# morriscb/chomp

Hardware: AMD Instinct MI355X
Metric: halo-model P(k,z) samples/sec (Stage K set-up + Stage E grid) (higher is better)
Workload: dtype f64

## Files before the change

### chomp_amd/csrc/chomp_capi.hip

```cpp
#include <hip/hip_runtime.h>

#include <dlfcn.h>

#include <algorithm>
#include <cmath>
#include <cstdio>
#include <cstddef>
#include <cstdint>
#include <cstdlib>
#include <cstring>
#include <string>
#include <map>
#include <unordered_map>
#include <vector>

#include "../../include/chomp_mi355x.h"
#include "chomp_power_kernels.h"
#include "chomp_proj_kernels.h"
#include "chomp_cov_kernels.h"
#include "chomp_probe_kernel.h"
#include "chomp_de_kernels.h"
#include "chomp_pt_kernels.h"
#include "chomp_tri_kernels.h"
#include "chomp_profile_kernels.h"
// ... 851 lines not shown
    return CHOMP_OK;
  if (n < 4 || n > 240) return fail(ctx, CHOMP_ERR_ARG, "dark energy: cosmo_npoints must be 4..240");
  if (nk > 65535) return fail(ctx, CHOMP_ERR_ARG, "dark energy: more than 65535 distinct (w0, wa)");
  T.valid = false;
  int rc = de_knots(ctx);
  if (rc) return rc;
  const DePar* before = T.d_par;
  rc = ensure(ctx, &T.d_par, &T.cap_par, nk);
  if (rc) return rc;
  if (T.d_par != before) T.sh_par.reset();
  rc = ensure(ctx, &T.d_tab, &T.cap_tab, nk * (size_t)de_stride(n));
  if (rc) return rc;
  rc = upload(ctx, T.d_par, keys.data(), nk * sizeof(DePar), T.sh_par);
  if (rc) return rc;
  hipLaunchKernelGGL(k_de_table, dim3((unsigned)n, (unsigned)nk), dim3(64 * kDeNW), 0, ctx->stream,
                     ctx->cfg, T.d_par, ctx->d_de_knots, T.d_tab);
  hipLaunchKernelGGL(k_de_spline, dim3((unsigned)nk), dim3(64), (size_t)(11 * n) * sizeof(double),
                     ctx->stream, ctx->cfg, T.d_tab);
  HIPCHK(hipGetLastError());
  T.keys = keys;
  T.valid = true;
  return CHOMP_OK;
}

int chomp_set_dark_energy(chomp_ctx* ctx, int on) {
  if (!ctx) return CHOMP_ERR_ARG;
  ctx->dark_energy = on != 0;
  return CHOMP_OK;
}

int chomp_set_general_profile(chomp_ctx* ctx, int on) {
  if (!ctx) return CHOMP_ERR_ARG;
  ctx->general_profile = on != 0;
  return CHOMP_OK;
}

int chomp_get_de_table(chomp_ctx* ctx, int source, size_t index, int what, double* out, size_t n) {
  if (!ctx || !out) return fail(ctx, CHOMP_ERR_ARG, "get_de_table: bad args");
  const int np = ctx->cfg.cosmo_npoints;
  int off;
  size_t want = (size_t)np;
  switch (what) {
    case CHOMP_DE_LN_A: off = de_off_ln_a(np); break;
    case CHOMP_DE_PRESSURE: off = de_off_p(np); break;
    case CHOMP_DE_LEVELS: off = de_off_level(np); break;
    case CHOMP_DE_CONVERGED: off = de_off_conv(np); break;
    case CHOMP_DE_PP: off = de_off_pp(np); want = 4 * (size_t)(np - 1); break;
    default: return fail(ctx, CHOMP_ERR_ARG, "get_de_table: unknown table part");
  }
  if (n != want) return fail(ctx, CHOMP_ERR_ARG, "get_de_table: n must be cosmo_npoints (4 (cosmo_npoints - 1) for the coefficients)");
  HIPCHK(hipSetDevice(ctx->device));
  const double* src;
  if (source == CHOMP_DE_EPOCH) {
    if (!ctx->have_epochs || index >= ctx->n_epoch) return fail(ctx, CHOMP_ERR_STATE, "get_de_table: epoch");
    if (index >= ctx->de_slot.size() || ctx->de_slot[index] < 0)
      return fail(ctx, CHOMP_ERR_STATE, "get_de_table: the epoch's cosmology has no dark energy");
    src = ctx->de_ep.d_tab + (size_t)ctx->de_slot[index] * de_stride(np);
  } else if (source == CHOMP_DE_PROJ) {
    if (!ctx->proj.me_ready || !ctx->proj.de)
      return fail(ctx, CHOMP_ERR_STATE, "get_de_table: no projection set-up with dark energy");
    { const int rcj = proj_join(ctx); if (rcj) return rcj; }
    src = ctx->de_proj.d_tab;
  } else {
    return fail(ctx, CHOMP_ERR_ARG, "get_de_table: unknown source");
  }
  HIPCHK(hipStreamSynchronize(ctx->stream));
  HIPCHK(hipMemcpy(out, src + off, n * sizeof(double), hipMemcpyDeviceToHost));
  return CHOMP_OK;
}

int chomp_epochs_set(chomp_ctx* ctx, size_t n_epoch, const chomp_cosmo* cosmo,
                     const double* z) {
  StageRange range_(ctx, "chomp:epochs_set (Stage K: sigma tables, mass-limit search)");
  if (!ctx || !cosmo || !z || n_epoch == 0) return fail(ctx, CHOMP_ERR_ARG, "epochs_set: bad args");
  for (size_t i = 0; i < n_epoch; ++i) {
    if (!ctx->dark_energy && has_dark_energy(cosmo[i].w0, cosmo[i].wa))
      return fail(ctx, CHOMP_ERR_SCOPE,
                  "w0 != -1 or wa != 0: dynamical dark energy (cosmology.py:96-104) needs "
                  "chomp_set_dark_energy(ctx, 1)");
    if (!(cosmo[i].omega_m0 > 0.0) || !(cosmo[i].h > 0.0) || !(cosmo[i].sigma_8 > 0.0))
      return fail(ctx, CHOMP_ERR_ARG, "epochs_set: omega_m0, h, sigma_8 must be > 0");
  }
  HIPCHK(hipSetDevice(ctx->device));
  int rc = alloc_epochs(ctx, n_epoch);
  if (rc) return rc;
  ctx->n_epoch = n_epoch;
  ctx->status_mirrored = false;
  { const int rch = ensure_hstatus(ctx); if (rch) return rch; }
  ctx->have_mass = ctx->have_halo = false;
  ctx->fam_mask = 0;
  ctx->put_mask.assign(n_epoch, 0u);
  ctx->delta_b_zero = true;
  ctx->have_halofit.assign(n_epoch, 0);
  ctx->tri_built.assign(n_epoch, 0);
  ctx->tri4_built.assign(n_epoch, 0);
  ctx->prof_general.assign(n_epoch, 0);
  rc = upload(ctx, ctx->d_cosmo, cosmo, n_epoch * sizeof(chomp_cosmo), ctx->sh_cosmo);
  if (rc) return rc;
  rc = upload(ctx, ctx->d_z, z, n_epoch * sizeof(double), ctx->sh_z);
  if (rc) return rc;
  std::vector<int> slot(n_epoch), first;
  {
    std::unordered_multimap<uint64_t, int> seen;
    seen.reserve(n_epoch * 2);
    for (size_t i = 0; i < n_epoch; ++i) {
      uint64_t h = 1469598103934665603ull;
      const unsigned char* b = reinterpret_cast<const unsigned char*>(&cosmo[i]);
      for (size_t j = 0; j < sizeof(chomp_cosmo); ++j) { h ^= b[j]; h *= 1099511628211ull; }
      int s_found = -1;
      auto range = seen.equal_range(h);
      for (auto it = range.first; it != range.second; ++it)
        if (std::memcmp(&cosmo[first[it->second]], &cosmo[i], sizeof(chomp_cosmo)) == 0) {
          s_found = it->second;
          break;
        }
      if (s_found < 0) {
        s_found = (int)first.size();
        first.push_back((int)i);
        seen.emplace(h, s_found);
      }
      slot[i] = s_found;
    }
  }
  const size_t n_slots = first.size();
  ctx->n_slots = n_slots;
  ctx->slot = slot;
  first.resize(n_epoch, 0);
  rc = upload(ctx, ctx->d_slot, slot.data(), n_epoch * sizeof(int), ctx->sh_slot);
  if (rc) return rc;
  rc = upload(ctx, ctx->d_first, first.data(), n_epoch * sizeof(int), ctx->sh_first);
  if (rc) return rc;
  std::vector<DePar> de_keys;
  ctx->de_slot.assign(n_epoch, -1);
  if (ctx->dark_energy) {
    std::map<std::pair<double, double>, int> seen;
    for (size_t i = 0; i < n_epoch; ++i) {
      if (!has_dark_energy(cosmo[i].w0, cosmo[i].wa)) continue;
      auto it = seen.emplace(std::make_pair(cosmo[i].w0, cosmo[i].wa), (int)de_keys.size());
      if (it.second) de_keys.push_back(DePar{cosmo[i].w0, cosmo[i].wa});
      ctx->de_slot[i] = it.first->second;
    }
  }
  const bool any_de = !de_keys.empty();
  if (any_de) {
    rc = de_build(ctx, ctx->de_ep, de_keys);
    if (rc) return rc;
    const int* before = ctx->d_de_slot;
    rc = ensure(ctx, &ctx->d_de_slot, &ctx->cap_de_slot, n_epoch);
    if (rc) return rc;
    if (ctx->d_de_slot != before) ctx->sh_de_slot.reset();
    rc = upload(ctx, ctx->d_de_slot, ctx->de_slot.data(), n_epoch * sizeof(int), ctx->sh_de_slot);
    if (rc) return rc;
  }
  const unsigned gy = (unsigned)(n_slots + (n_epoch + 255) / 256);
  rc = with_flag(ctx->with_bao, n_slots >= 16, [&](auto BAO, auto MANY) {
    constexpr int NPT = MANY ? 4 : 1;
    hipLaunchKernelGGL((k_sigma_nodes<BAO, NPT>),
                       dim3(sigma_node_blocks<NPT>() + sigma_lns_blocks<NPT>() + sigma_gtab_blocks<NPT>(), gy),
                       dim3(256), 0, ctx->stream, ctx->cfg, ctx->d_cosmo, ctx->d_z, ctx->d_first,
                       ctx->d_slot, (int)n_slots, (int)n_epoch, ctx->d_epochs, ctx->d_snodes,
                       ctx->d_status);
    if (!MANY) return CHOMP_OK;
    const size_t shl = BAO ? 0 : (size_t)kGTabCount * sizeof(double);
    if constexpr (!BAO) {
      const int rcl = lds_opt_in(ctx, &k_sigma_lns<BAO>, (int)shl);
      if (rcl) return rcl;
    }
    hipLaunchKernelGGL(k_sigma_lns<BAO>, dim3((unsigned)n_slots), dim3(kLnsThreads), shl, ctx->stream,
                       ctx->cfg, ctx->d_cosmo, ctx->d_z, ctx->d_first, ctx->d_snodes);
    return CHOMP_OK;
  });
  if (rc) return rc;
  if (any_de)
    hipLaunchKernelGGL(k_de_epochs, dim3((unsigned)((n_epoch + 63) / 64)), dim3(64), 0, ctx->stream,
                       ctx->cfg, ctx->d_de_slot, (int)n_epoch, ctx->de_ep.d_tab, ctx->d_epochs,
                       ctx->d_status);
  if (n_epoch >= 128)
    with_flag(ctx->with_bao, [&](auto BAO) {
      hipLaunchKernelGGL((k_epoch_probe<BAO, 1, 1>), dim3((unsigned)n_epoch, 2 * kProbes), dim3(64), 0,
                         ctx->stream, ctx->cfg, ctx->d_epochs, ctx->d_search, ctx->d_cand, ctx->d_snodes,
                         ctx->d_probe, ctx->d_count, ctx->d_status);
    });
  chomp::launch_epoch_probe(ctx->with_bao != 0, (unsigned)n_epoch, ctx->stream, ctx->cfg,
                            ctx->d_epochs, ctx->d_search, ctx->d_cand, ctx->d_snodes,
                            ctx->d_probe, ctx->d_count, ctx->d_status);
  if (any_de)
    hipLaunchKernelGGL(k_de_chi, dim3((unsigned)n_epoch), dim3(64), 0, ctx->stream, ctx->cfg,
                       ctx->d_de_slot, ctx->de_ep.d_tab, ctx->d_epochs);
  HIPCHK(hipGetLastError());
  ctx->have_epochs = true;
  return CHOMP_OK;
}

struct HaloPlan {
  unsigned fam = 0, kmask = 0;
  int groups[4] = {-1, -1, -1, -1};
  int ng = 0;
  int want_nbar = 1;
  bool eval = false;
  bool general = false;
  bool has_hod() const {
    return group_hod(groups[0]) || group_hod(groups[1]) || group_hod(groups[2]) ||
           group_hod(groups[3]);
  }
};
static std::vector<chomp_hod_model> zheng_models(const chomp_hod_par* hod, size_t n) {
  std::vector<chomp_hod_model> m(n);
  for (size_t i = 0; i < n; ++i) {
    m[i] = chomp_hod_model{};
    m[i].kind = CHOMP_HOD_ZHENG;
    m[i].zheng = hod[i];
  }
  return m;
}
static_assert(kHodZheng == CHOMP_HOD_ZHENG && kHodMandelbaum == CHOMP_HOD_MANDELBAUM,
              "chomp_math.h's model numbers are the header's");
static_assert(PT_FS2 == CHOMP_PT_FS2 && PT_FS2_LEN == CHOMP_PT_FS2_LEN &&
                  PT_FS2_KDIFF == CHOMP_PT_FS2_KDIFF && PT_FS3 == CHOMP_PT_FS3 &&
                  PT_FS3_PARALLELOGRAM == CHOMP_PT_FS3_PARALLELOGRAM && PT_F3 == CHOMP_PT_F3 &&
                  PT_FS3_BCGS == CHOMP_PT_FS3_BCGS && PT_BISPECTRUM == CHOMP_PT_BISPECTRUM &&
                  PT_BISPECTRUM_LEN == CHOMP_PT_BISPECTRUM_LEN &&
                  PT_TRISPECTRUM == CHOMP_PT_TRISPECTRUM &&
                  PT_TRISPECTRUM_PARALLELOGRAM == CHOMP_PT_TRISPECTRUM_PARALLELOGRAM &&
                  kPtForms == CHOMP_PT_TRISPECTRUM_PARALLELOGRAM + 1,
              "chomp_pt_kernels.h's form numbers are the header's");
static int halo_prepare(chomp_ctx* ctx, const chomp_halo_par* profile, const chomp_hod_model* hod,
                        unsigned tables, HaloPlan* P) {
  const size_t n = ctx->n_epoch;
  for (size_t i = 0; i < n; ++i) {
    if (profile[i].alpha == -1.0) continue;
    if (!ctx->general_profile)
      return fail(ctx, CHOMP_ERR_SCOPE,
                  "halo alpha != -1: the general-profile transform y_general "
                  "(halo.py:491-559) is outside the hot-path scope (NFW only) unless "
                  "chomp_set_general_profile(ctx, 1)");
    if (!(profile[i].alpha > -3.0) || !(profile[i].alpha <= kProfileAlphaMax))
      return fail(ctx, CHOMP_ERR_ARG, "halo_setup: alpha must lie in (-3, 3.5]");
    P->general = true;
  }
  for (size_t i = 0; i < n; ++i)
    if ((hod[i].kind != CHOMP_HOD_ZHENG && hod[i].kind != CHOMP_HOD_MANDELBAUM) ||
        hod[i].reserved != 0)
      return fail(ctx, CHOMP_ERR_ARG, "halo_setup: unknown HOD model");
  std::vector<HodDev> hd(n);
  for (size_t i = 0; i < n; ++i) {
    HodDev& d = hd[i];
    d.model = hod[i].kind;
    d.pad_ = 0;
    d.w = 0.0;
    d.M_min = 0.0;
    if (hod[i].kind == CHOMP_HOD_MANDELBAUM) {
      d.log_M_0 = hod[i].log_M_0;
      mandelbaum_constants(hod[i].log_M_0, &d.log_M_min, &d.M_min);
      d.w = hod[i].w;
      d.sigma = 0.0; d.log_M_1p = 0.0; d.alpha = 1.0;
      d.first_zero = d.second_zero = d.safe_norm = -1.0;
      continue;
    }
    const chomp_hod_par& h = hod[i].zheng;
    d.log_M_min = h.log_M_min; d.sigma = h.sigma; d.log_M_0 = h.log_M_0;
    d.log_M_1p = h.log_M_1p; d.alpha = h.alpha;
    d.first_zero = std::pow(10.0, h.log_M_min +
                                      h.sigma * erfinv_host(2.0 * ctx->cfg.halo_precision - 1.0));
    d.second_zero = std::pow(10.0, h.log_M_0);
    d.safe_norm = std::pow(10.0, h.log_M_min + 1.0 * h.sigma);
    if (h.alpha != 1.0) P->eval = true;
  }
  int rcu = upload(ctx, ctx->d_profile, profile, n * sizeof(chomp_halo_par), ctx->sh_profile);
  if (rcu) return rcu;
  rcu = upload(ctx, ctx->d_hod, hd.data(), n * sizeof(HodDev), ctx->sh_hod);
  if (rcu) return rcu;
  P->fam = tables & ((1u << kFamilies) - 1u);
  P->kmask = P->fam | ((tables & CHOMP_T_EXCLUSION) ? kMaskExclusion : 0u);
  P->ng = 0;
  if (P->fam & ((1u << F_HM) | (1u << F_PPMM))) P->groups[P->ng++] = 0;
  if (P->fam & ((1u << F_HG) | (1u << F_PPGM))) P->groups[P->ng++] = 1;
  if (P->fam & (1u << F_PPGG)) P->groups[P->ng++] = 2;
  if (P->fam & (1u << F_I12)) P->groups[P->ng++] = 3;
  if (P->has_hod() && ctx->cfg.divmax > kNodeLevel)
    P->kmask |= kMaskDeepNodes;
  return CHOMP_OK;
}

static int launch_nu_mass(chomp_ctx* ctx, int mf_kind, const HaloPlan* plan) {
  ctx->status_mirrored = false;
  const size_t n = ctx->n_epoch;
  const TabLayout& L = ctx->L;
  const int ef = (ctx->n_slots < 16 || n > 65535) ? 1 : 0;
  ctx->have_b2 = false;
  if (ctx->second_order) {
    ctx->B2 = make_b2_layout(L.NM);
    const int rcb = ensure(ctx, &ctx->d_b2, &ctx->cap_b2, n * (size_t)ctx->B2.stride);
    if (rcb) return rcb;
  }
  with_flag(ctx->with_bao, (size_t)L.NM * n <= 512, [&](auto BAO, auto FEW) {
    constexpr int NW = FEW ? 4 : 1;
    const dim3 grid = ef ? dim3((unsigned)n, L.NM) : dim3(L.NM, (unsigned)n);
    if (ctx->second_order)
      hipLaunchKernelGGL((k_nu_table<BAO, NW, true>), grid, dim3(64 * NW), 0, ctx->stream, ctx->cfg,
                         L, ctx->d_epochs, ctx->d_search, ctx->d_snodes, ctx->d_tab, ctx->d_status,
                         ef, ctx->d_b2, ctx->B2.stride);
    else
      hipLaunchKernelGGL((k_nu_table<BAO, NW>), grid, dim3(64 * NW), 0, ctx->stream, ctx->cfg, L,
                         ctx->d_epochs, ctx->d_search, ctx->d_snodes, ctx->d_tab, ctx->d_status, ef,
                         nullptr, 0);
  });
  const size_t sh = (size_t)mass_lds_doubles(L.NM) * sizeof(double);
  const int ng = plan && plan->ng > 0 ? plan->ng : 1;
  unsigned chunks = plan ? (unsigned)(512 / (n * ng)) : 1u;
  chunks = chunks < 1 ? 1 : (chunks > 12 ? 12 : chunks);
  hipLaunchKernelGGL(k_mass_nodes, dim3((unsigned)n, (unsigned)ng, chunks), dim3(256), sh, ctx->stream,
                     ctx->cfg, L, ctx->d_epochs, ctx->d_search, ctx->d_tab, ctx->d_mass_par, mf_kind,
                     ctx->d_tinker, ctx->d_gl16, plan ? 1 : 0, ctx->d_profile, ctx->d_hod,
                     ctx->d_sici, ctx->d_nodes, ctx->d_endp, plan ? plan->groups[0] : -1,
                     plan ? plan->groups[1] : -1, plan ? plan->groups[2] : -1,
                     plan ? plan->groups[3] : -1, plan ? plan->kmask : 0u, ctx->d_status, ctx->d_npend, ctx->d_pending);
  if (ctx->second_order) {
    hipLaunchKernelGGL(k_mass_b2, dim3((unsigned)n), dim3(64 * kB2NW),
                       (size_t)b2_lds_doubles(L.NM) * sizeof(double), ctx->stream, ctx->cfg, L,
                       ctx->B2, ctx->d_epochs, ctx->d_tab, ctx->d_b2, ctx->d_status);
    ctx->have_b2 = true;
  }
  HIPCHK(hipGetLastError());
  return CHOMP_OK;
}

extern "C++" struct KnotsFast {
  chomp_ctx* ctx;
  const HaloPlan& P;
  size_t lds;
// ... 1162 lines not shown
```

### chomp_amd/csrc/chomp_mass_kernels.h

```cpp
#pragma once

#include <type_traits>

#include <hip/hip_runtime.h>

#include "../../include/chomp_mi355x.h"
#include "chomp_math.h"
#include "chomp_romberg.h"

namespace chomp {

enum { F_HM = 0, F_PPMM = 1, F_HG = 2, F_PPGM = 3, F_PPGG = 4, F_I12 = 5 };
constexpr int kFamilies = 6;

struct TabLayout {
  int NM, NK;
  int off_ln_mass, off_nu, off_nu_pp, off_lnm_pp;
  int off_knot[6], off_kpp[6];
  int off_levels, off_hf_lns2, off_misc;
  int stride;
  unsigned long long* h_status;
  unsigned h_seq;
};

// ... 55 lines not shown
__device__ __forceinline__ void copy_doubles(double* dst, const double* src, int n) {
  for (int i = threadIdx.x; i < n; i += blockDim.x) dst[i] = src[i];
}

constexpr int kSigmaLevel = 13;
constexpr int kSigmaCount = (1 << kSigmaLevel) + 1;
constexpr int kSGrid = 48;
struct SGrid {
  double b0, b1, b2, b3, b4;
  bool valid;
  __host__ __device__ void segment(double x, double* lo, double* hi, int* n, int* off) const {
    if (x <= b1) { *lo = b0; *hi = b1; *n = 8; *off = 0; }
    else if (x <= b2) { *lo = b1; *hi = b2; *n = 14; *off = 8; }
    else if (x <= b3) { *lo = b2; *hi = b3; *n = 18; *off = 22; }
    else { *lo = b3; *hi = b4; *n = 8; *off = 40; }
  }
  __host__ __device__ double ln_r(int i) const {
    double lo, hi;
    int n, off;
    if (i < 8) { lo = b0; hi = b1; n = 8; off = 0; }
    else if (i < 22) { lo = b1; hi = b2; n = 14; off = 8; }
    else if (i < 40) { lo = b2; hi = b3; n = 18; off = 22; }
    else { lo = b3; hi = b4; n = 8; off = 40; }
    return lo + (hi - lo) * (double)(i - off) / (double)(n - 1);
  }
};
__host__ __device__ inline SGrid make_sgrid(double k_min, double k_max) {
  SGrid g;
  const double a = log(14.0662 / k_max) - log(100.0), b = log(14.0662 / k_max),
               c = log(0.1 / k_min);
  g.b0 = a - log(20.0);
  g.b1 = a; g.b2 = b; g.b3 = c;
  g.b4 = c + log(3.0);
  g.valid = b < c;
  return g;
}
constexpr int kSigmaOffI8 = 2 * kSigmaCount, kSigmaOffLnS = 2 * kSigmaCount + 8;
constexpr int kSigmaNodeBlocks = (kSigmaCount + 255) / 256;
constexpr int kSigmaOffPart = kSigmaOffLnS + kSGrid;
constexpr int kSigmaOffG = kSigmaOffPart + kSigmaNodeBlocks * (kSigmaLevel + 1);
constexpr int kGTabN = 8192;
constexpr int kGTabPad = 3;
static_assert(kGTabN == kGTabIntervals, "chomp_math.h: epoch_k_range");
constexpr int kGTabCount = kGTabN + 1 + 2 * kGTabPad;
constexpr int kGTabBlocks = (kGTabCount + 255) / 256;
constexpr int kSigmaStride = kSigmaOffG + 2 * kGTabCount;

struct SigmaInterpIntegrand {
  UniformDoubles g;
  double xlo, dx, inv_dx;
  double scale, amp2_nine_over_r6, amp2;
  bool tiny_r;
  SinCosLead lead = sincos_lead();
  __device__ __forceinline__ double operator()(double ln_k) const {
    const double u = (ln_k - xlo) * inv_dx;
    int i = (int)u;
    i = i < 0 ? 0 : (i > kGTabN - 1 ? kGTabN - 1 : i);
    const double t = u - (double)i;
    UniformDoubles q = g + i + kGTabPad - 2;
    const double a = t + 2.0, b = t + 1.0, d = t - 1.0, e = t - 2.0, f = t - 3.0;
    const double ab = a * b, ef = e * f, cd = t * d;
    const double gv = q[0] * (b * cd * ef) * (-1.0 / 120.0) + q[1] * (a * cd * ef) * (1.0 / 24.0) +
                      q[2] * (ab * d * ef) * (-1.0 / 12.0) + q[3] * (ab * t * ef) * (1.0 / 12.0) +
                      q[4] * (ab * cd * f) * (-1.0 / 24.0) + q[5] * (ab * cd * e) * (1.0 / 120.0);
    const double y = t * dx;
    const double ey = fma(y, fma(y, fma(y, fma(y, 1.0 / 24.0, 1.0 / 6.0), 0.5), 1.0), 1.0);
    const double k = q[2 + kGTabCount] * ey;
    const double kR = scale * k;
    if (tiny_r) {
      double s, c;
      fast_sincos_pm(kR, &s, &c);
      const double kR2 = kR * kR, k3 = k * k * k;
      const double W = 3.0 * (s / (kR2 * kR) - c / kR2);
      return amp2 * (gv * (k3 * k3)) * (W * W);
    }
    const double w = tophat_numer_pm(kR, lead);
    return amp2_nine_over_r6 * gv * (w * w);
  }
};

template <bool BAO>
__device__ __forceinline__ void sigma8_from_parts(const chomp_config& cfg, const Epoch& E,
                                                  double* __restrict__ n, int nb, double* red) {
  const double a = log(cfg.k_min), b = log(cfg.k_max);
  const bool tab8 = 0.1 / 8.0 > cfg.k_min && 14.0662 / 8.0 < cfg.k_max && cfg.divmax >= 1;
  __shared__ double stage[kSigmaNodeBlocks * (kSigmaLevel + 1)];
  __shared__ double S[kSigmaLevel + 1];
  __shared__ double i8;
  __shared__ int converged;
  for (int q = threadIdx.x; q < nb * (kSigmaLevel + 1); q += blockDim.x)
    stage[q] = __hip_atomic_load(n + kSigmaOffPart + q, __ATOMIC_RELAXED, __HIP_MEMORY_SCOPE_AGENT);
  __syncthreads();
  if (threadIdx.x <= kSigmaLevel) {
    double t = 0.0;
    for (int q = 0; q < nb; ++q) t += stage[q * (kSigmaLevel + 1) + threadIdx.x];
    S[threadIdx.x] = t;
  }
  __syncthreads();
  if (threadIdx.x < 64) {
    const int lane = threadIdx.x;
    const double range = b - a;
    double ordsum = 0.5 * S[0], nn = 1.0;
    double result = range * ordsum, prev = result;
    double Tl = lane == 0 ? result : 0.0;
    int conv = 0;
    const int top = cfg.divmax < kSigmaLevel ? cfg.divmax : kSigmaLevel;
    double crow[kSigmaLevel + 1];
#pragma unroll
    for (int i = 1; i <= kSigmaLevel; ++i) crow[i] = CHOMP_ROMBERG_C[i][lane & 31];
#pragma unroll
    for (int i = 1; i <= kSigmaLevel; ++i) {
      if (tab8 && i <= top && !conv) {
        nn *= 2.0;
        ordsum += S[i];
        const double Ti = ldexp(range * ordsum, -i);
        if (lane == i) Tl = Ti;
        result = wave_sum32(crow[i] * Tl);
        const double err = fabs(result - prev);
        prev = result;
        if (err < cfg.global_precision || err < cfg.cosmo_precision * fabs(result)) conv = 1;
      }
    }
    if (tab8 && !conv && cfg.divmax <= kSigmaLevel) conv = 1;
    if (lane == 0) {
      converged = conv;
      i8 = result;
    }
  }
  __syncthreads();
  if (!converged) {
    double lo, hi;
    sigma_limits(E, 8.0, &lo, &hi);
    SigmaIntegrandT<BAO> f{&E, 8.0};
    double s2;
    if (blockDim.x == 256) {
      s2 = romberg1<4>(f, lo, hi, cfg.global_precision, cfg.cosmo_precision, cfg.divmax, red);
    } else {
      s2 = 0.0;
      if (threadIdx.x < 64)
        s2 = romberg1<1>(f, lo, hi, cfg.global_precision, cfg.cosmo_precision, cfg.divmax, nullptr);
    }
    if (threadIdx.x == 0) i8 = s2;
  }
  if (threadIdx.x == 0) n[kSigmaOffI8] = i8;
}

template <int NPT>
__host__ __device__ constexpr int sigma_node_blocks() { return (kSigmaCount + 256 * NPT - 1) / (256 * NPT); }
template <int NPT>
__host__ __device__ constexpr int sigma_lns_blocks() { return NPT == 1 ? kSGrid : 0; }
template <int NPT>
__host__ __device__ constexpr int sigma_gtab_blocks() { return (kGTabCount + 256 * NPT - 1) / (256 * NPT); }

template <bool BAO, int NPT>
__global__ __launch_bounds__(256) void k_sigma_nodes(chomp_config cfg,
                                                     const chomp_cosmo* __restrict__ cosmo,
                                                     const double* __restrict__ zin,
                                                     const int* __restrict__ first,
                                                     const int* __restrict__ slots, int n_slots,
                                                     int n_epoch, Epoch* __restrict__ epochs,
                                                     double* __restrict__ snodes,
                                                     unsigned* __restrict__ status) {
  static_assert(NPT == 1 || NPT == 4, "nodes per thread");
  static_assert(kSGrid % 4 == 0, "four ln S points to a block");
  __shared__ Epoch E;
  __shared__ double red[romberg_scratch<4, 1>()];
  if ((int)blockIdx.y >= n_slots) {
    const int e = ((int)blockIdx.y - n_slots) * 256 + (int)threadIdx.x;
    if (blockIdx.x != 0 || e >= n_epoch) return;
    Epoch B;
    double* q = reinterpret_cast<double*>(&B);
    for (int i = 0; i < kEpochDoubles; ++i) q[i] = 0.0;
    const chomp_cosmo c = cosmo[e];
    B.om0 = c.omega_m0; B.ob0 = c.omega_b0; B.ol0 = c.omega_l0; B.or0 = c.omega_r0;
    B.tcmb = c.cmb_temp; B.h = c.h; B.sigma8 = c.sigma_8; B.ns = c.n_scalar;
    B.z = zin[e];
    epoch_background(B, cfg.cosmo_precision, cfg.k_min, cfg.k_max, BAO ? 1 : 0);
    B.cosmo_slot = slots[e];
    epochs[e] = B;
    status[e] = 0u;
    return;
  }
  const int slot = blockIdx.y, e = first[slot];
  constexpr int nb = sigma_node_blocks<NPT>();
  constexpr int nl = sigma_lns_blocks<NPT>();
  if (threadIdx.x == 0) {
    const chomp_cosmo c = cosmo[e];
    E.om0 = c.omega_m0; E.ob0 = c.omega_b0; E.ol0 = c.omega_l0; E.or0 = c.omega_r0;
    E.tcmb = c.cmb_temp; E.h = c.h; E.sigma8 = c.sigma_8; E.ns = c.n_scalar;
    E.z = zin[e];
    epoch_shape_only(E, cfg.k_min, cfg.k_max, BAO ? 1 : 0);
  }
  __syncthreads();
  double* n = snodes + (size_t)slot * kSigmaStride;
  if ((int)blockIdx.x >= nb + nl) {
    const double xlo = log(cfg.k_min / 100.0), xhi = log(cfg.k_max * 100.0);
#pragma unroll
    for (int r = 0; r < NPT; ++r) {
      const int i = (((int)blockIdx.x - nb - nl) * NPT + r) * 256 + (int)threadIdx.x;
      if (i < kGTabCount) {
        const double x = xlo + (xhi - xlo) * ((double)(i - kGTabPad) / (double)kGTabN);
        const double k = exp(x);
        const double T = transfer_t<BAO>(E, k);
        const double k3 = k * k * k;
        n[kSigmaOffG + i] = exp((3.0 + E.ns) * (x - E.ln_H0)) * T * T / (k3 * k3);
        n[kSigmaOffG + kGTabCount + i] = k;
      }
    }
    return;
  }
  if ((int)blockIdx.x >= nb) {
    const int i = (int)blockIdx.x - nb;
    const double R = exp(make_sgrid(cfg.k_min, cfg.k_max).ln_r(i));
    double lo, hi;
    sigma_limits(E, R, &lo, &hi);
    SigmaIntegrandT<BAO> f{&E, R};
    const double s2 = romberg1<4>(f, lo, hi, cfg.global_precision, 1e-5,
                                  cfg.divmax < 10 ? cfg.divmax : 10, red);
    if (threadIdx.x == 0) n[kSigmaOffLnS + i] = log(s2);
    return;
  }
  const double a = log(cfg.k_min), b = log(cfg.k_max);
  const bool tab8 = 0.1 / 8.0 > cfg.k_min && 14.0662 / 8.0 < cfg.k_max && cfg.divmax >= 1;
  __shared__ double wsum[4][kSigmaLevel + 1];
  __shared__ int last_block;
  const int wv = threadIdx.x >> 6;
  if ((threadIdx.x & 63) <= kSigmaLevel) wsum[wv][threadIdx.x & 63] = 0.0;
#pragma unroll
  for (int r = 0; r < NPT; ++r) {
    const int first_idx = ((int)blockIdx.x * NPT + r) * 256;
    const int idx = first_idx + (int)threadIdx.x;
    const bool live = idx < kSigmaCount;
    int lev = 0;
    double g = 0.0;
    if (live) {
      double x;
      if (idx < 2) {
        x = idx == 0 ? a : b;
      } else {
        const int m = idx - 1;
        lev = 32 - __builtin_clz((unsigned)m);
        const long j = m - (1 << (lev - 1));
        const double h = ldexp(b - a, 1 - lev);
        x = (a + 0.5 * h) + h * (double)j;
      }
      const double k = exp(x);
      const double T = transfer_t<BAO>(E, k);
      n[idx] = k;
      const double k3 = k * k * k;
      const double d2k6 = exp((3.0 + E.ns) * (x - E.ln_H0)) * T * T / (k3 * k3);
      n[kSigmaCount + idx] = d2k6;
      const double t = tophat_numer_pm(8.0 * k);
      g = d2k6 * (9.0 / 262144.0) * (t * t);
    }
    if (first_idx < kSigmaCount) {
      const int last_idx = first_idx + 255;
      const int lev_lo = first_idx < 2 ? 0 : 32 - __builtin_clz((unsigned)(first_idx - 1));
      const int lev_hi = last_idx < 2 ? 0 : 32 - __builtin_clz((unsigned)(last_idx - 1));
      for (int l = lev_lo; l <= lev_hi && l <= kSigmaLevel; ++l) {
        const double v = wave_sum(live && lev == l ? g : 0.0);
        if ((threadIdx.x & 63) == 0) wsum[wv][l] += v;
      }
    }
  }
  double* part = n + kSigmaOffPart + (size_t)blockIdx.x * (kSigmaLevel + 1);
  __syncthreads();
  if (threadIdx.x <= kSigmaLevel) {
    __hip_atomic_store(part + threadIdx.x,
                       ((wsum[0][threadIdx.x] + wsum[1][threadIdx.x]) + wsum[2][threadIdx.x]) +
                           wsum[3][threadIdx.x],
                       __ATOMIC_RELAXED, __HIP_MEMORY_SCOPE_AGENT);
    asm volatile("s_waitcnt vmcnt(0)" ::: "memory");
  }
  if constexpr (NPT != 1) {
    return;
  } else {
    int* arrivals = reinterpret_cast<int*>(n + kSigmaOffI8 + 1);
    __syncthreads();
    if (threadIdx.x == 0) last_block = atomicAdd(arrivals, 1) == nb - 1 ? 1 : 0;
    __syncthreads();
    if (!last_block) return;
    if (threadIdx.x == 0) *arrivals = 0;
    sigma8_from_parts<BAO>(cfg, E, n, nb, red);
  }
}

struct SigmaInterpLds {
  static constexpr bool kLaneMajor = true;
  static constexpr bool kGeometric = true;
  const double* g;
  double xlo, dx, inv_dx, scale, nine_over_r6;
  bool tiny_r;
  SinCosLead lead = sincos_lead();
  __device__ __forceinline__ double operator()(double ln_k) const { return with_exp(ln_k, exp(ln_k)); }
  __device__ __forceinline__ double with_exp(double ln_k, double k) const {
    const double u = (ln_k - xlo) * inv_dx;
    int i = (int)u;
    i = i < 0 ? 0 : (i > kGTabN - 1 ? kGTabN - 1 : i);
    const double t = u - (double)i;
    const double* q = g + i + kGTabPad - 2;
    const double a = t + 2.0, b = t + 1.0, d = t - 1.0, e = t - 2.0, f = t - 3.0;
    const double ab = a * b, ef = e * f, cd = t * d;
    const double gv = q[0] * (b * cd * ef) * (-1.0 / 120.0) + q[1] * (a * cd * ef) * (1.0 / 24.0) +
                      q[2] * (ab * d * ef) * (-1.0 / 12.0) + q[3] * (ab * t * ef) * (1.0 / 12.0) +
                      q[4] * (ab * cd * f) * (-1.0 / 24.0) + q[5] * (ab * cd * e) * (1.0 / 120.0);
    const double kR = scale * k;
    if (tiny_r) {
      double s, c;
      fast_sincos_pm(kR, &s, &c);
      const double kR2 = kR * kR, k3 = k * k * k;
      const double W = 3.0 * (s / (kR2 * kR) - c / kR2);
      return (gv * (k3 * k3)) * (W * W);
    }
    const double w = tophat_numer_pm(kR, lead);
    return nine_over_r6 * gv * (w * w);
  }
};

constexpr int kLnsThreads = 512;
// ... 225 lines not shown
    int jl = seed_dir == 0 ? 0 : seed_jl, jh = seed_dir == 0 ? -1 : seed_jh;
    double tl = dir < 0 ? log(nu0 / thr) : log(thr / nu0);
    double th = jh < 0 ? 0.0 : (dir < 0 ? log(nu_h / thr) : log(thr / nu_h));
    double d = (side == 0 ? 0.25 : 0.7) * 0.04879;
    for (int it = 0; it < 4 * kSearchJ; ++it) {
      int jp;
      if (jh < 0) {
        double want = ceil(tl / d);
        if (!(want >= 1.0)) want = 1.0;
        if (want > 256.0) want = 256.0;
        jp = jl + (int)want;
        if (jp > kSearchJ - 1) jp = kSearchJ - 1;
      } else {
        if (jh == jl + 1) break;
        const double dd = (tl - th) / (double)(jh - jl);
        double want = ceil(tl / dd);
        if (!(want >= 1.0)) want = 1.0;
        if (want > (double)(jh - jl - 1)) want = (double)(jh - jl - 1);
        jp = jl + (int)want;
      }
      const double nu = nu_probe<NW, BAO>(E, snode, tab[jp], cfg, T.thr_lo, T.thr_hi, red);
      ++*n_eval;
      const bool pred = dir < 0 ? !(thr < nu) : !(thr > nu);
      const double tp = dir < 0 ? log(nu / thr) : log(thr / nu);
      if (pred) {
        jh = jp;
        th = tp;
      } else {
        if (jh < 0) {
          const double dn = (tl - tp) / (double)(jp - jl);
          d = dn > 1e-6 ? dn : 1e-6;
        }
        jl = jp;
        tl = tp;
        if (jh < 0 && jp == kSearchJ - 1) { jh = jp; *exhausted = true; break; }
      }
    }
    if (jh < 0) jh = jl;
    mass = tab[jh];
  }
  return mass;
}

__device__ __forceinline__ unsigned search_status(const Epoch& E, int side, double mass,
                                                  bool exhausted) {
  const double R = scale_of_mass(E, mass);
  unsigned st = 0u;
  if (side == 0 && 100.0 * E.k_max * R < 0.2) st |= kStMassMinSaturated;
  if (side == 1 && 0.1 / R <= E.k_min / 100.0) st |= kStMassMaxSaturated;
  if (exhausted) st |= kStSearchExhausted;
  return st;
}

__device__ __forceinline__ double ln_s_estimate(const SGrid& G, const double* lns, double x) {
  if (!G.valid || !(x >= G.b0 && x <= G.b4)) return NAN;
  double lo, hi;
  int n, off;
  G.segment(x, &lo, &hi, &n, &off);
  const double u = (x - lo) / (hi - lo) * (double)(n - 1);
  int i0 = (int)floor(u) - 2;
  i0 = i0 < 0 ? 0 : (i0 > n - 6 ? n - 6 : i0);
  const double* f = lns + off + i0;
  const double t = u - (double)i0;
  const double t0 = t, t1 = t - 1.0, t2 = t - 2.0, t3 = t - 3.0, t4 = t - 4.0, t5 = t - 5.0;
  return f[0] * (t1 * t2 * t3 * t4 * t5) * (-1.0 / 120.0) +
         f[1] * (t0 * t2 * t3 * t4 * t5) * (1.0 / 24.0) +
         f[2] * (t0 * t1 * t3 * t4 * t5) * (-1.0 / 12.0) +
         f[3] * (t0 * t1 * t2 * t4 * t5) * (1.0 / 12.0) +
         f[4] * (t0 * t1 * t2 * t3 * t5) * (-1.0 / 24.0) +
         f[5] * (t0 * t1 * t2 * t3 * t4) * (1.0 / 120.0);
}

struct SidePlan {
  bool ok;
  int dir, j;
  double nu_start;
  bool at_edge;
};
__device__ __forceinline__ SidePlan plan_side(const Epoch& E, const double* lns, int side,
                                              const double* cand, int* sh) {
  const SideThresholds T = side_thresholds(side, cand);
  const SGrid G = make_sgrid(E.k_min, E.k_max);
  const double margin = 1e-2;
  const double ln_margin = 0.00995033085;
  SidePlan P{false, 0, 0, 0.0, false};
  const int lane = threadIdx.x & 63;
  const double arg = lane == 0 ? E.delta_c * E.delta_c / (E.amp * E.sigma_norm * E.sigma_norm)
                   : lane == 1 ? 3.0 * T.down[0] / (4.0 * kPi * E.rho_bar)
                   : lane == 2 ? T.thr_hi : T.thr_lo;
  const double lg = log(arg);
  const double ln_nu_c = readlane_d(lg, 0), x0 = readlane_d(lg, 1) * (1.0 / 3.0);
  const double ln_hi = readlane_d(lg, 2), ln_lo = readlane_d(lg, 3);
  const double step = 0.016263388 ;
  const double ln_nu0 = ln_nu_c - ln_s_estimate(G, lns, x0);
  P.nu_start = exp(ln_nu0);
  if (!(ln_nu0 == ln_nu0)) return P;
  if (ln_nu0 > ln_hi + ln_margin) P.dir = -1;
  else if (ln_nu0 < ln_lo - ln_margin) P.dir = +1;
  else if (ln_nu0 >= ln_lo + ln_margin && ln_nu0 <= ln_hi - ln_margin) {
    P.ok = true;
    return P;
  } else {
    P.ok = true;
    P.at_edge = true;
    P.dir = P.nu_start > 0.5 * (T.thr_lo + T.thr_hi) ? -1 : +1;
    P.j = 2;
    return P;
  }
  (void)margin;
  const double ln_thr = P.dir < 0 ? ln_hi : ln_lo;
  auto passes = [&](int j) {
    const double ln_nu = ln_nu_c - ln_s_estimate(G, lns, x0 + (double)(P.dir * j) * step);
    return !(ln_nu == ln_nu) || (P.dir < 0 ? !(ln_thr < ln_nu) : !(ln_thr > ln_nu));
  };
  constexpr int kStride = kSearchJ / 256;
  __syncthreads();
  if (threadIdx.x == 0) *sh = kSearchJ;
  __syncthreads();
  for (int t = (int)threadIdx.x; t < 256; t += (int)blockDim.x) {
    const int j = kStride * (1 + t) - 1;
    if (j < kSearchJ && passes(j)) atomicMin(sh, j);
  }
  __syncthreads();
  const int jc = *sh;
  __syncthreads();
  if (jc < kSearchJ && (int)threadIdx.x < kStride - 1) {
    const int j = jc - (kStride - 1) + (int)threadIdx.x;
    if (j >= 1 && passes(j)) atomicMin(sh, j);
  }
  __syncthreads();
  const int j = *sh;
  if (j >= kSearchJ) return P;
  const double lsj = ln_s_estimate(G, lns, x0 + (double)(P.dir * j) * step);
  if (!(lsj == lsj)) return P;
  P.j = j;
  P.ok = true;
  return P;
}

template <class F>
decltype(auto) with_flag(bool flag, F&& f) {
  return flag ? f(std::true_type{}) : f(std::false_type{});
}
template <class F>
decltype(auto) with_flag(bool a, bool b, F&& f) {
  return with_flag(a, [&](auto A) { return with_flag(b, [&](auto B) { return f(A, B); }); });
}
template <int N>
using int_c = std::integral_constant<int, N>;

void launch_epoch_probe(bool bao, unsigned n_epoch, hipStream_t stream, const chomp_config& cfg,
                        Epoch* epochs, double* search, const double* cand, const double* snodes,
                        double* probe, int* count, unsigned* status);
constexpr int kProbes = 4;
constexpr int kProbeStride = 24;

template <bool BAO, int NW, bool SIG = false>
__global__ __launch_bounds__(64 * NW) void k_nu_table(chomp_config cfg, TabLayout L,
                                                      const Epoch* __restrict__ epochs,
                                                      const double* __restrict__ search,
                                                      const double* __restrict__ snodes,
                                                      double* __restrict__ tab,
                                                      unsigned* __restrict__ status,
                                                      int epochs_fastest,
                                                      double* __restrict__ sig = nullptr,
                                                      int sig_stride = 0) {
  __shared__ Epoch E;
  __shared__ double red[romberg_scratch<NW, 1>()];
  int e = epochs_fastest ? (int)blockIdx.x : (int)blockIdx.y;
  int i = (int)blockIdx.x;
  if (!epochs_fastest) {
    const int NM = (int)gridDim.x, n = (int)gridDim.y;
    const int b = (int)blockIdx.x + NM * (int)blockIdx.y;
    if (b < 8 * NM * (n / 8)) {
      const int slot = b >> 3;
      e = (slot / NM) * 8 + (b & 7);
      i = slot % NM;
    }
  }
  if (epochs_fastest) {
    const int NM = (int)gridDim.y, y = (int)blockIdx.y, m0 = NM / 2 - 1;
    if (NM < 8) i = NM - 1 - y;
    else if (y < 2) i = m0 + y;
    else if (y >= NM - 2) i = m0 + 2 + (y - (NM - 2));
    else { i = NM - 1 - (y - 2); if (i <= m0 + 3) i -= 4; }
  }
  copy_doubles(reinterpret_cast<double*>(&E), reinterpret_cast<const double*>(&epochs[e]),
               kEpochDoubles);
  __syncthreads();
  const double* snode = snodes + (size_t)E.cosmo_slot * kSigmaStride;
  const double ln_lo = search[(e * 2 + 0) * 2], ln_hi = search[(e * 2 + 1) * 2];
  const double lnm = linspace_at(ln_lo, ln_hi, L.NM, i);
  bool conv = true;
  double nu;
  if constexpr (SIG) {
    const double s2 = sigma2_block<NW, 1, BAO>(E, snode, scale_of_mass(E, exp(lnm)), cfg,
                                               cfg.cosmo_precision, red, &conv);
    const double sq = E.delta_c / sqrt(s2);
    nu = sq * sq;
    if (threadIdx.x == 0) sig[(size_t)e * sig_stride + i] = sqrt(s2);
  } else {
    nu = nu_of_mass_block<NW, 1, BAO>(E, snode, exp(lnm), cfg, cfg.cosmo_precision, red, &conv);
  }
  if (threadIdx.x == 0) {
    double* t = tab + (size_t)e * L.stride;
    t[L.off_ln_mass + i] = lnm;
    t[L.off_nu + i] = nu;
    if (!conv) atomicOr(&status[e], kStSigmaDivmax);
  }
}

struct TinkerTab {
  double x[9];
  double c[5][32];
};

struct FnuLn {
  const Epoch* e;
  __device__ __forceinline__ double operator()(double t) const {
    const double nu = exp(t);
    return f_nu(*e, nu) * nu;
  }
};
struct FnuLin {
  const Epoch* e;
  __device__ __forceinline__ double operator()(double nu) const { return f_nu(*e, nu); }
};
struct FnuBiasLin {
  const Epoch* e;
  __device__ __forceinline__ double operator()(double nu) const {
    return f_nu(*e, nu) * bias_nu(*e, nu);
  }
};
constexpr int kNormLiteralDivmax = 18;
struct FnuBiasLn {
  const Epoch* e;
  __device__ __forceinline__ double operator()(double t) const {
    const double nu = exp(t);
    return f_nu(*e, nu) * bias_nu(*e, nu) * nu;
  }
};

struct MassLds {
  double *x_lnm, *y_nu, *c_nu, *c_lnm, *work, *gl, *red;
  __device__ __forceinline__ void carve(double* sm, int NM) {
    x_lnm = sm;
    y_nu = x_lnm + NM;
    c_nu = y_nu + NM;
    c_lnm = c_nu + 4 * (NM - 1);
    work = c_lnm + 4 * (NM - 1);
    gl = work + 18 * NM;
    red = gl + 32;
  }
};
__host__ __device__ inline int mass_lds_doubles(int NM) {
  return 2 * NM + 8 * (NM - 1) + 18 * NM + 32 + romberg_scratch<4, 2>();
}

template <class Beside>
__device__ __forceinline__ void mass_setup_block(
    const chomp_config& cfg, const TabLayout& L, Epoch& E, Epoch* __restrict__ epochs, int e,
    bool publish, double ln_mass_min, double ln_mass_max, int n_search, double* __restrict__ t,
    const chomp_halo_par& hp, int mf_kind, const TinkerTab* __restrict__ tinker,
    const double* __restrict__ gl16, const MassLds& M, Beside&& beside) {
  const int NM = L.NM;
  copy_doubles(M.x_lnm, t + L.off_ln_mass, NM);
  copy_doubles(M.y_nu, t + L.off_nu, NM);
  copy_doubles(M.gl, gl16, 32);
  __syncthreads();
  {
    const int sys = threadIdx.x >> 7, tid = threadIdx.x & 127;
    spline_build_pcr(sys == 0 ? M.x_lnm : M.y_nu, sys == 0 ? M.y_nu : M.x_lnm, NM,
                     sys == 0 ? M.c_nu : M.c_lnm, M.work + sys * 9 * NM, tid, 128, true);
  }
  if (threadIdx.x < 64) {
    const int lane = (int)threadIdx.x;
    const double mf_delta_v = (hp.delta_v == -1.0) ? E.delta_v : hp.delta_v;
    double mine = 0.0;
    if (mf_kind == CHOMP_MF_TINKER && lane < 5) {
      const double ld = log(mf_delta_v);
      const double opz = 1.0 + E.z;
      mine = spline_eval(tinker->x, tinker->c[lane], 9, ld);
      const double ex = lane == 1 ? 0.20 : (lane == 2 ? -0.01 : (lane == 3 ? -0.08 : 0.27));
      if (lane > 0) mine *= pow(opz, ex);
    }
    if (lane == 5) mine = exp(spline_eval(M.y_nu, M.c_lnm, NM, 1.0));
    const double t_alpha = readlane_d(mine, 0), t_beta = readlane_d(mine, 1);
    const double t_gamma = readlane_d(mine, 2), t_phi = readlane_d(mine, 3);
    const double t_eta = readlane_d(mine, 4), m_star = readlane_d(mine, 5);
    if (lane == 0) {
      E.ln_mass_min = ln_mass_min;
      E.ln_mass_max = ln_mass_max;
      E.n_search = n_search;
      E.nu_min = 1.001 * M.y_nu[0];
      E.nu_max = 0.999 * M.y_nu[NM - 1];
      E.m_star = m_star;
      E.stq = hp.stq;
      E.st_a = hp.st_little_a;
      E.mf_delta_v = mf_delta_v;
      E.mf_kind = mf_kind;
      E.f_norm = 1.0;
      E.bias_norm = 1.0;
      E.ln_st_a = log(hp.st_little_a);
      E.ln_t_beta = 0.0;
      if (mf_kind == CHOMP_MF_TINKER) {
        E.t_alpha = t_alpha;
        E.t_beta = t_beta;
        E.t_gamma = t_gamma;
// ... 59 lines not shown
```

### chomp_amd/csrc/chomp_probe.hip

```cpp
#include <hip/hip_runtime.h>

#include "../../include/chomp_mi355x.h"
#include "chomp_probe_kernel.h"

namespace chomp {

void launch_epoch_probe(bool bao, unsigned n_epoch, hipStream_t stream, const chomp_config& cfg,
                        Epoch* epochs, double* search, const double* cand, const double* snodes,
                        double* probe, int* count, unsigned* status) {
  const bool large = n_epoch >= 128;
  const dim3 grid = large ? dim3(n_epoch) : dim3(n_epoch, 2 * kProbes);
  with_flag(bao, large, [&](auto BAO, auto LARGE) {
    hipLaunchKernelGGL((k_epoch_probe<BAO, LARGE ? 2 : 0>), grid, dim3(64 * kInitNW), 0, stream,
                       cfg, epochs, search, cand, snodes, probe, count, status);
  });
}

}
```

### chomp_amd/csrc/chomp_probe_kernel.h

```cpp
#pragma once

#include "chomp_mass_kernels.h"

namespace chomp {

template <bool BAO, int PHASE, int NW = kInitNW>
__global__ __launch_bounds__(64 * NW, NW == 1 ? 4 : 1) void k_epoch_probe(
    chomp_config cfg, Epoch* __restrict__ epochs, double* __restrict__ search,
    const double* __restrict__ cand, const double* __restrict__ snodes,
    double* __restrict__ probe, int* __restrict__ count, unsigned* __restrict__ status) {
  __shared__ Epoch E;
  __shared__ double red[romberg_scratch<NW, 1>()];
  __shared__ double lns[kSGrid];
  __shared__ int last, sh_j;
  __shared__ double seeds[2][6];
  __shared__ int open_side[2];
  const int e = blockIdx.x, role = PHASE == 2 ? 0 : 2 * kProbes - 1 - (int)blockIdx.y;
  const bool chi_role = PHASE != 2 && role == kProbes;
  const int side = role / kProbes, p = role % kProbes;
  const bool fixed = cfg.mass_min > 0.0 && cfg.mass_max > 0.0;
  if (fixed && !chi_role) return;
  copy_doubles(reinterpret_cast<double*>(&E), reinterpret_cast<const double*>(&epochs[e]),
               kEpochDoubles);
  __syncthreads();
  const double* snode = snodes + (size_t)E.cosmo_slot * kSigmaStride;
  copy_doubles(lns, snode + kSigmaOffLnS, kSGrid);
  if (threadIdx.x == 0) {
    E.sigma_norm = E.sigma8 * E.growth / sqrt(E.amp * snode[kSigmaOffI8]);
  }
  __syncthreads();
  double* pr = probe + (size_t)e * kProbeStride;
  if (chi_role) {
    EIntegrand f{E.om0, E.ol0, E.or0, E.H0};
    const double chi = romberg1<NW>(f, 0.0, E.z, cfg.global_precision,
                                         cfg.cosmo_precision, cfg.divmax, red);
    __syncthreads();
    if (threadIdx.x == 0) {
      E.chi = chi;
      __hip_atomic_store(pr + 2 * kProbes, chi, __ATOMIC_RELAXED, __HIP_MEMORY_SCOPE_AGENT);
    }
    __syncthreads();
    if (fixed) {
      if (threadIdx.x == 0) {
        search[(e * 2 + 0) * 2 + 0] = log(cfg.mass_min);
        search[(e * 2 + 0) * 2 + 1] = 0.0;
        search[(e * 2 + 1) * 2 + 0] = log(cfg.mass_max);
        search[(e * 2 + 1) * 2 + 1] = 0.0;
      }
      __syncthreads();
      copy_doubles(reinterpret_cast<double*>(&epochs[e]), reinterpret_cast<const double*>(&E),
                   kEpochDoubles);
      return;
    }
  }
  if constexpr (PHASE != 2) {
    const SidePlan plan = plan_side(E, lns, side, cand, &sh_j);
    const SideThresholds T = side_thresholds(side, cand);
    double nu_mine = NAN;
    if (plan.ok && plan.dir != 0) {
      const int c = plan.j - 2 + p;
      if ((c > 0 || (c == 0 && plan.at_edge)) && c < kSearchJ) {
        const double* tab = plan.dir < 0 ? T.down : T.up;
        nu_mine = nu_probe<NW, BAO>(E, snode, tab[c], cfg, T.thr_lo, T.thr_hi, red);
      }
    }
    if (threadIdx.x == 0) {
      auto put = [](double* q, double v) {
        __hip_atomic_store(q, v, __ATOMIC_RELAXED, __HIP_MEMORY_SCOPE_AGENT);
      };
      put(pr + role, nu_mine);
      if (p == 0) {
        double* pl = pr + 2 * kProbes + 4 + 4 * side;
        put(pl, plan.ok ? (plan.at_edge ? 2.0 : 1.0) : 0.0);
        put(pl + 1, (double)plan.dir);
        put(pl + 2, (double)plan.j);
        put(pl + 3, plan.nu_start);
      }
    }
  }
  if constexpr (PHASE != 1) {
  if constexpr (PHASE == 0) {
    if (threadIdx.x == 0) {
      asm volatile("s_waitcnt vmcnt(0)" ::: "memory");
      last = atomicAdd(&count[e], 1) == 2 * kProbes - 1 ? 1 : 0;
    }
    __syncthreads();
    if (!last) return;
  }
  __shared__ double rec[kProbeStride];
  if (threadIdx.x < kProbeStride)
    rec[threadIdx.x] = __hip_atomic_load(pr + threadIdx.x, __ATOMIC_RELAXED, __HIP_MEMORY_SCOPE_AGENT);
  __syncthreads();
  if (threadIdx.x < 2) {
    auto peek = [&](const double* q) { return rec[q - pr]; };
    {
      const int sd = (int)threadIdx.x;
      const double* pl = pr + 2 * kProbes + 4 + 4 * sd;
      const double mode = peek(pl);
      const bool ok = mode != 0.0, at_edge = mode == 2.0;
      const int dir = (int)peek(pl + 1);
      const int j = (int)peek(pl + 2);
      double nu_start = peek(pl + 3);
      const SideThresholds S = side_thresholds(sd, cand);
      double mass = S.down[0];
      int n_eval = 0;
      bool certified = ok;
      int seed_dir = 0, seed_jl = 0, seed_jh = -1;
      double nu_l = 0.0, nu_h = 0.0;
      bool walk = ok && dir != 0;
      if (at_edge) {
        nu_start = peek(pr + kProbes * sd);
        const int dir_exact = S.thr_hi < nu_start ? -1 : (S.thr_lo > nu_start ? +1 : 0);
        n_eval = 1;
        if (!(nu_start == nu_start)) { certified = false; walk = false; n_eval = 0; }
        else if (dir_exact == 0) walk = false;
        else if (dir_exact != dir) {
          certified = false; walk = false;
          seed_dir = dir_exact; seed_jl = 0; nu_l = nu_start;
        }
      }
      if (walk) {
        const double* tab = dir < 0 ? S.down : S.up;
        const double thr = dir < 0 ? S.thr_hi : S.thr_lo;
        int st0, st1, st2, st3;
        double nu0, nu1, nu2, nu3;
        auto classify = [&](int q, int* st, double* nu) {
          const int c = j - 2 + q;
          *nu = peek(pr + kProbes * sd + q);
          if (c <= 0) *st = 0;
          else if (!(*nu == *nu)) *st = -1;
          else { *st = (dir < 0 ? !(thr < *nu) : !(thr > *nu)) ? 1 : 0; ++n_eval; }
        };
        classify(0, &st0, &nu0); classify(1, &st1, &nu1);
        classify(2, &st2, &nu2); classify(3, &st3, &nu3);
        certified = false;
        int first_pass = -1, before = -1;
        double nu_first = 0.0;
        if (st3 == 1) { first_pass = 3; nu_first = nu3; before = st2; }
        if (st2 == 1) { first_pass = 2; nu_first = nu2; before = st1; }
        if (st1 == 1) { first_pass = 1; nu_first = nu1; before = st0; }
        if (st0 == 1) { first_pass = 0; nu_first = nu0; before = -1; }
        if (first_pass > 0 && before == 0) {
          certified = true;
          mass = tab[j - 2 + first_pass];
        } else if (first_pass == 0 && j - 2 == 1) {
          certified = true;
          mass = tab[1];
        }
        if (!certified) {
          seed_dir = dir;
          seed_jl = 0; nu_l = nu_start;
          if (st0 == 0 && j - 2 > 0) { seed_jl = j - 2; nu_l = nu0; }
          if (st1 == 0 && j - 1 > 0) { seed_jl = j - 1; nu_l = nu1; }
          if (st2 == 0 && j > 0) { seed_jl = j; nu_l = nu2; }
          if (st3 == 0 && j + 1 > 0) { seed_jl = j + 1; nu_l = nu3; }
          if (first_pass >= 0 && j - 2 + first_pass > seed_jl) {
            seed_jh = j - 2 + first_pass; nu_h = nu_first;
          }
        }
      }
      seeds[sd][0] = (double)seed_dir; seeds[sd][1] = (double)seed_jl; seeds[sd][2] = nu_l;
      seeds[sd][3] = (double)seed_jh; seeds[sd][4] = nu_h; seeds[sd][5] = (double)n_eval;
      open_side[sd] = certified ? 0 : 1;
      if (certified) {
        search[(e * 2 + sd) * 2 + 0] = log(mass);
        search[(e * 2 + sd) * 2 + 1] = (double)n_eval;
        const unsigned st = search_status(E, sd, mass, false);
        if (st) atomicOr(&status[e], st);
      }
    }
    if (threadIdx.x == 0) {
      E.chi = peek(pr + 2 * kProbes);
      if (PHASE == 0) count[e] = 0;
    }
  }
  __syncthreads();
  for (int sd = 0; sd < 2; ++sd) {
    if (!open_side[sd]) continue;
    int n_eval = (int)seeds[sd][5];
    bool exhausted = false;
    const double mass = search_side_exact<NW, BAO>(
        E, snode, sd, cfg, cand, red, &n_eval, &exhausted, (int)seeds[sd][0], (int)seeds[sd][1],
        seeds[sd][2], (int)seeds[sd][3], seeds[sd][4]);
    if (threadIdx.x == 0) {
      search[(e * 2 + sd) * 2 + 0] = log(mass);
      search[(e * 2 + sd) * 2 + 1] = (double)n_eval;
      const unsigned st = search_status(E, sd, mass, exhausted);
      if (st) atomicOr(&status[e], st);
    }
  }
  __syncthreads();
  copy_doubles(reinterpret_cast<double*>(&epochs[e]), reinterpret_cast<const double*>(&E),
// ... 6 lines not shown
```

Measured before the change: 2.290 billion.

## Compute comoving distance inside sigma-node kernel for small epoch batches

For batches below the large-batch threshold, extra grid rows are added to the sigma-node kernel so that each epoch's comoving-distance Romberg integral runs there and is written into the probe buffer. The small-batch probe kernel (PHASE 0) then reads that value instead of integrating it again, which moves the chi integration off the probe kernel's critical path and overlaps it with the sigma-node work. In exchange the sigma-node grid grows, and the chi value is computed from the raw cosmology with a hardcoded H0 constant and a clamped z. That could differ slightly from the Epoch-based computation it replaces.

```diff
diff --git a/chomp_amd/csrc/chomp_capi.hip b/chomp_amd/csrc/chomp_capi.hip
--- a/chomp_amd/csrc/chomp_capi.hip
+++ b/chomp_amd/csrc/chomp_capi.hip
@@ -1027,14 +1027,16 @@
     rc = upload(ctx, ctx->d_de_slot, ctx->de_slot.data(), n_epoch * sizeof(int), ctx->sh_de_slot);
     if (rc) return rc;
   }
-  const unsigned gy = (unsigned)(n_slots + (n_epoch + 255) / 256);
+  const bool chi_here = n_epoch < (size_t)kProbeLargeBatch;
   rc = with_flag(ctx->with_bao, n_slots >= 16, [&](auto BAO, auto MANY) {
     constexpr int NPT = MANY ? 4 : 1;
-    hipLaunchKernelGGL((k_sigma_nodes<BAO, NPT>),
-                       dim3(sigma_node_blocks<NPT>() + sigma_lns_blocks<NPT>() + sigma_gtab_blocks<NPT>(), gy),
+    constexpr int gx = sigma_node_blocks<NPT>() + sigma_lns_blocks<NPT>() + sigma_gtab_blocks<NPT>();
+    const unsigned gy = (unsigned)(n_slots + sigma_epoch_rows((int)n_epoch) +
+                                   (chi_here ? sigma_chi_rows((int)n_epoch, gx) : 0));
+    hipLaunchKernelGGL((k_sigma_nodes<BAO, NPT>), dim3(gx, gy),
                        dim3(256), 0, ctx->stream, ctx->cfg, ctx->d_cosmo, ctx->d_z, ctx->d_first,
                        ctx->d_slot, (int)n_slots, (int)n_epoch, ctx->d_epochs, ctx->d_snodes,
-                       ctx->d_status);
+                       ctx->d_status, chi_here ? ctx->d_probe : nullptr);
     if (!MANY) return CHOMP_OK;
     const size_t shl = BAO ? 0 : (size_t)kGTabCount * sizeof(double);
     if constexpr (!BAO) {
@@ -1050,7 +1052,7 @@
     hipLaunchKernelGGL(k_de_epochs, dim3((unsigned)((n_epoch + 63) / 64)), dim3(64), 0, ctx->stream,
                        ctx->cfg, ctx->d_de_slot, (int)n_epoch, ctx->de_ep.d_tab, ctx->d_epochs,
                        ctx->d_status);
-  if (n_epoch >= 128)
+  if (n_epoch >= (size_t)kProbeLargeBatch)
     with_flag(ctx->with_bao, [&](auto BAO) {
       hipLaunchKernelGGL((k_epoch_probe<BAO, 1, 1>), dim3((unsigned)n_epoch, 2 * kProbes), dim3(64), 0,
                          ctx->stream, ctx->cfg, ctx->d_epochs, ctx->d_search, ctx->d_cand, ctx->d_snodes,
diff --git a/chomp_amd/csrc/chomp_mass_kernels.h b/chomp_amd/csrc/chomp_mass_kernels.h
--- a/chomp_amd/csrc/chomp_mass_kernels.h
+++ b/chomp_amd/csrc/chomp_mass_kernels.h
@@ -231,6 +231,15 @@
 template <int NPT>
 __host__ __device__ constexpr int sigma_gtab_blocks() { return (kGTabCount + 256 * NPT - 1) / (256 * NPT); }
 
+constexpr int kProbes = 4;
+constexpr int kProbeStride = 24;
+constexpr int kProbeLargeBatch = 128;
+
+__host__ __device__ constexpr int sigma_epoch_rows(int n_epoch) { return (n_epoch + 255) / 256; }
+__host__ __device__ constexpr int sigma_chi_rows(int n_epoch, int blocks_x) {
+  return (n_epoch + blocks_x - 1) / blocks_x;
+}
+
 template <bool BAO, int NPT>
 __global__ __launch_bounds__(256) void k_sigma_nodes(chomp_config cfg,
                                                      const chomp_cosmo* __restrict__ cosmo,
@@ -239,11 +248,24 @@
                                                      const int* __restrict__ slots, int n_slots,
                                                      int n_epoch, Epoch* __restrict__ epochs,
                                                      double* __restrict__ snodes,
-                                                     unsigned* __restrict__ status) {
+                                                     unsigned* __restrict__ status,
+                                                     double* __restrict__ probe) {
   static_assert(NPT == 1 || NPT == 4, "nodes per thread");
   static_assert(kSGrid % 4 == 0, "four ln S points to a block");
   __shared__ Epoch E;
   __shared__ double red[romberg_scratch<4, 1>()];
+  if ((int)blockIdx.y >= n_slots + sigma_epoch_rows(n_epoch)) {
+    const int e = ((int)blockIdx.y - n_slots - sigma_epoch_rows(n_epoch)) * (int)gridDim.x +
+                  (int)blockIdx.x;
+    if (e >= n_epoch) return;
+    const chomp_cosmo c = cosmo[e];
+    const double z = zin[e] < 0.0 ? 0.0 : zin[e];
+    EIntegrand f{c.omega_m0, c.omega_l0, c.omega_r0, 100.0 / (2.998 * 100000.0)};
+    const double chi = romberg1<4>(f, 0.0, z, cfg.global_precision, cfg.cosmo_precision,
+                                   cfg.divmax, red);
+    if (threadIdx.x == 0) probe[(size_t)e * kProbeStride + 2 * kProbes] = chi;
+    return;
+  }
   if ((int)blockIdx.y >= n_slots) {
     const int e = ((int)blockIdx.y - n_slots) * 256 + (int)threadIdx.x;
     if (blockIdx.x != 0 || e >= n_epoch) return;
@@ -775,8 +797,6 @@
 void launch_epoch_probe(bool bao, unsigned n_epoch, hipStream_t stream, const chomp_config& cfg,
                         Epoch* epochs, double* search, const double* cand, const double* snodes,
                         double* probe, int* count, unsigned* status);
-constexpr int kProbes = 4;
-constexpr int kProbeStride = 24;
 
 template <bool BAO, int NW, bool SIG = false>
 __global__ __launch_bounds__(64 * NW) void k_nu_table(chomp_config cfg, TabLayout L,
diff --git a/chomp_amd/csrc/chomp_probe.hip b/chomp_amd/csrc/chomp_probe.hip
--- a/chomp_amd/csrc/chomp_probe.hip
+++ b/chomp_amd/csrc/chomp_probe.hip
@@ -8,7 +8,7 @@
 void launch_epoch_probe(bool bao, unsigned n_epoch, hipStream_t stream, const chomp_config& cfg,
                         Epoch* epochs, double* search, const double* cand, const double* snodes,
                         double* probe, int* count, unsigned* status) {
-  const bool large = n_epoch >= 128;
+  const bool large = n_epoch >= (unsigned)kProbeLargeBatch;
   const dim3 grid = large ? dim3(n_epoch) : dim3(n_epoch, 2 * kProbes);
   with_flag(bao, large, [&](auto BAO, auto LARGE) {
     hipLaunchKernelGGL((k_epoch_probe<BAO, LARGE ? 2 : 0>), grid, dim3(64 * kInitNW), 0, stream,
diff --git a/chomp_amd/csrc/chomp_probe_kernel.h b/chomp_amd/csrc/chomp_probe_kernel.h
--- a/chomp_amd/csrc/chomp_probe_kernel.h
+++ b/chomp_amd/csrc/chomp_probe_kernel.h
@@ -30,14 +30,19 @@
   }
   __syncthreads();
   double* pr = probe + (size_t)e * kProbeStride;
-  if (chi_role) {
-    EIntegrand f{E.om0, E.ol0, E.or0, E.H0};
-    const double chi = romberg1<NW>(f, 0.0, E.z, cfg.global_precision,
-                                         cfg.cosmo_precision, cfg.divmax, red);
-    __syncthreads();
+  if (chi_role && (PHASE != 0 || fixed)) {
+    double chi;
+    if constexpr (PHASE == 0) {
+      chi = pr[2 * kProbes];
+    } else {
+      EIntegrand f{E.om0, E.ol0, E.or0, E.H0};
+      chi = romberg1<NW>(f, 0.0, E.z, cfg.global_precision, cfg.cosmo_precision, cfg.divmax, red);
+      __syncthreads();
+    }
     if (threadIdx.x == 0) {
       E.chi = chi;
-      __hip_atomic_store(pr + 2 * kProbes, chi, __ATOMIC_RELAXED, __HIP_MEMORY_SCOPE_AGENT);
+      if (PHASE != 0)
+        __hip_atomic_store(pr + 2 * kProbes, chi, __ATOMIC_RELAXED, __HIP_MEMORY_SCOPE_AGENT);
     }
     __syncthreads();
     if (fixed) {
```

Result: faster. 2.317 billion (median of 6 runs) (+1.2%).
